# masnottuh/point-cloud-toolbox

Measured on AMD Instinct MI355X. Metric: points/sec curvature (1M-pt torus, k=50); HBM GB/s k-NN vs peak, higher is better.
Workload: dtype f64

## Files before the change

### point-cloud-toolbox_amd/csrc/pct_api.hip

```cpp
#include "pct_internal.h"
#include "pct_auto_route.h"
#include "pct_query_plan.h"
#include "pct_ball_plan.h"

#include <execinfo.h>
#include <math.h>
#include <mutex>
#include <signal.h>
#include <stdarg.h>
#include <stdlib.h>
#include <sys/prctl.h>
#include <unistd.h>

int pct_fail(pct_ctx* ctx, int code, const char* fmt, ...) {
    if (ctx) {
        va_list ap;
        va_start(ap, fmt);
        vsnprintf(ctx->err, sizeof(ctx->err), fmt, ap);
        va_end(ap);
    }
    return code;
}

extern char** environ;
// ... 182 lines not shown
    }
    for (auto& e : ctx->ev)
        if (hipEventCreate(&e) != hipSuccess) {
            delete ctx;
            return PCT_ERR_HIP;
        }
    for (int i = PCT_EV_CALL_BEGIN; i <= PCT_EV_FAST_END; ++i)
        if (hipEventCreate(&ctx->ev_prev[i]) != hipSuccess) {
            delete ctx;
            return PCT_ERR_HIP;
        }
    if (hipHostMalloc((void**)&ctx->pin, 4096, hipHostMallocMapped) != hipSuccess) {
        delete ctx;
        return PCT_ERR_OOM;
    }
    memset(ctx->pin, 0, 4096);
    if (hipDeviceGetAttribute(&ctx->clock_khz, hipDeviceAttributeWallClockRate, device) != hipSuccess || ctx->clock_khz < 0) ctx->clock_khz = 0;
    (void)hipGetLastError();
    *out = ctx;
    return PCT_OK;
}

void pct_destroy(pct_ctx* ctx) {
    if (!ctx) return;
    (void)hipSetDevice(ctx->device);
    if (ctx->stream) (void)hipStreamSynchronize(ctx->stream);
    pct_comm_release(ctx);
    pct_buf* all[] = {&ctx->xyz, &ctx->pts4, &ctx->pts4d, &ctx->cell_of, &ctx->cell_cnt, &ctx->cell_fill,
                      &ctx->scan_tmp, &ctx->occ, &ctx->redo, &ctx->row_of, &ctx->owned_pos, &ctx->cell_own, &ctx->cell_oth, &ctx->own_start, &ctx->sorted4, &ctx->sorted4d, &ctx->red, &ctx->nbr_pos,
                      &ctx->nbr_dist, &ctx->nbr_cnt, &ctx->counters, &ctx->coefs, &ctx->K, &ctx->H, &ctx->H2,
                      &ctx->stage_a, &ctx->stage_b, &ctx->stage_c, &ctx->stage_d, &ctx->row_done, &ctx->redo_m, &ctx->flag_buf, &ctx->dens_buf, &ctx->pub_pos, &ctx->pub_dist, &ctx->pub_cnt, &ctx->qpts4, &ctx->qry, &ctx->ball_off, &ctx->ball_idx, &ctx->ball_alt, &ctx->ball_dist, &ctx->fit_flag, &ctx->lvl_src,
                      &ctx->tree_codes, &ctx->tree_vals, &ctx->tree_lvl, &ctx->tree_head, &ctx->tree_marks, &ctx->tree_seg, &ctx->tree_runs, &ctx->tree_range, &ctx->tree_bucket, &ctx->tree_tmp,
                      &ctx->pca, &ctx->pca_aux, &ctx->pca_nbr, &ctx->pca_orig,
                      &ctx->bin_rec, &ctx->bin_mat, &ctx->bin_plan, &ctx->bin_base,
                      &ctx->area, &ctx->area_closed, &ctx->area_nverts, &ctx->area_over, &ctx->stamp_tickets};
    for (pct_buf* b : all) pct_release(b);
    if (ctx->pin) (void)hipHostFree(ctx->pin);
    for (auto& e : ctx->ev)
        if (e) (void)hipEventDestroy(e);
    for (auto& e : ctx->ev_prev)
        if (e) (void)hipEventDestroy(e);
    if (ctx->stream) (void)hipStreamDestroy(ctx->stream);
    delete ctx;
}

const char* pct_last_error(const pct_ctx* ctx) { return ctx ? ctx->err : "null context"; }

static int begin_call(pct_ctx* ctx, bool wait_for_pending = true) {
    if (!ctx) return PCT_ERR_INVALID;
    ctx->err[0] = 0;
    PCT_HIP(ctx, hipSetDevice(ctx->device));
    if (wait_for_pending) PCT_TRY(drain(ctx));
    return PCT_OK;
}

static int new_cloud(pct_ctx* ctx, int64_t n) {
    if (n <= 0 || n > (int64_t)INT32_MAX - 1024) return pct_fail(ctx, PCT_ERR_INVALID, "cloud size %lld out of range", (long long)n);
    ctx->n = n;
    ctx->q_begin = 0;
    ctx->q_end = n;
    ctx->slab_parts = ctx->slab_part = 0;
    ctx->slab_split_valid = false;
    ctx->grid_valid = ctx->knn_valid = ctx->fit_valid = ctx->pts4_valid = ctx->qpts4_valid = false;
    ctx->pca_valid = false;
    ctx->ball_valid = false;
    ctx->area_valid = false;
    ctx->has_f64 = false;
// ... 1202 lines not shown
```

### point-cloud-toolbox_amd/csrc/pct_grid.hip

```cpp
#include "pct_internal.h"
#include "pct_grid_edge.h"

#include <math.h>
#include <stdlib.h>

namespace {

constexpr int kBlock = 256;

__device__ __forceinline__ float wave_min(float v) {
    for (int o = 32; o > 0; o >>= 1) v = fminf(v, __shfl_xor(v, o));
    return v;
}
__device__ __forceinline__ float wave_max(float v) {
    for (int o = 32; o > 0; o >>= 1) v = fmaxf(v, __shfl_xor(v, o));
    return v;
}

struct PackRed {
    int bb[6];
    int bad;
    int g_begin;
    double s[3], ss[3];
    unsigned long long cnt;
// ... 798 lines not shown
__global__ __launch_bounds__(kBinWide) void k_bin_scatter(const float* __restrict__ xyz, const float4* __restrict__ pts4, int64_t n,
                                                           int tile_rows, pct_grid g, int shift, int nb, int chunk,
                                                           const unsigned* __restrict__ mat, const int* __restrict__ plan,
                                                           float4* __restrict__ rec, int* __restrict__ cell_own, int* __restrict__ cell_oth) {
    __shared__ unsigned s_cur[kBinMaxBuckets];
    const int* bstart = plan + 16;
    for (int b = threadIdx.x; b < nb; b += kBinWide) s_cur[b] = (unsigned)bstart[b] + mat[(size_t)blockIdx.x * nb + b];
    __syncthreads();
    const int64_t r0 = (int64_t)blockIdx.x * tile_rows, r1 = min(n, r0 + tile_rows);
    for (int64_t base = r0 + threadIdx.x; base < r1; base += 4 * kBinWide) {
        float4 p[4];
#pragma unroll
        for (int j = 0; j < 4; ++j)
            if (base + j * kBinWide < r1) p[j] = bin_load<RAW>(xyz, pts4, base + j * kBinWide);
#pragma unroll
        for (int j = 0; j < 4; ++j) {
            if (base + j * kBinWide >= r1) continue;
            const unsigned pos = atomicAdd(&s_cur[bin_cell(p[j].x, p[j].y, p[j].z, g) >> shift], 1u);
            if (pos < (unsigned)n) rec[pos] = p[j];
        }
    }
    if (plan[2] > 0) {
        for (int b = blockIdx.x; b < nb; b += gridDim.x) {
            if (bstart[b + 1] - bstart[b] <= chunk) continue;
            const int64_t c0 = (int64_t)b << shift, c1 = min(g.ncell, c0 + ((int64_t)1 << shift));
            for (int64_t c = c0 + threadIdx.x; c < c1; c += kBinWide) {
                cell_own[c] = 0;
                if (cell_oth) cell_oth[c] = 0;
            }
        }
    }
}

__global__ __launch_bounds__(kBinBlock) void k_bin_cells(const float4* __restrict__ rec, const int* __restrict__ plan,
                                                         const int4* __restrict__ items, pct_grid g, int shift, int q_begin, int q_end,
                                                         int* __restrict__ cell_own, int* __restrict__ cell_oth, int* __restrict__ base,
                                                         const PackRed* __restrict__ parts, int n_parts, PackRed* __restrict__ red,
                                                         PackRed* __restrict__ red_host) {
    extern __shared__ int s_c[];
    if (blockIdx.x == gridDim.x - 1) {
        if (parts) pack_fold<kBinBlock>(parts, n_parts, red, red_host, 0);
        return;
    }
    if ((int)blockIdx.x >= plan[0]) return;
    const int4 it = items[blockIdx.x];
    const int r0 = it.y, r1 = it.z, slot = it.w;
    const int cpb = 1 << shift, nc = cell_oth ? 2 * cpb : cpb;
    const int64_t c0 = (int64_t)it.x << shift;
    const int ncl = (int)min((int64_t)cpb, g.ncell - c0);
    for (int k = threadIdx.x; k < nc; k += kBinBlock) s_c[k] = 0;
    __syncthreads();
    for (int base = r0 + threadIdx.x; base < r1; base += 4 * kBinBlock) {
        float4 p[4];
#pragma unroll
        for (int j = 0; j < 4; ++j)
            if (base + j * kBinBlock < r1) p[j] = rec[base + j * kBinBlock];
#pragma unroll
        for (int j = 0; j < 4; ++j) {
            if (base + j * kBinBlock >= r1) continue;
            const int l = bin_cell(p[j].x, p[j].y, p[j].z, g) - (int)c0;
            const int idx = __float_as_int(p[j].w);
            const bool owned = !cell_oth || (idx >= q_begin && idx < q_end);
            if ((unsigned)l < (unsigned)cpb) atomicAdd(&s_c[(owned ? 0 : cpb) + l], 1);
        }
    }
    __syncthreads();
    for (int k = threadIdx.x; k < nc; k += kBinBlock) {
        const int l = k & (cpb - 1);
        if (l >= ncl) continue;
        int* arr = k < cpb ? cell_own : cell_oth;
        const int v = s_c[k];
        if (slot < 0) arr[c0 + l] = v;
        else base[(size_t)slot * nc + k] = v ? atomicAdd(&arr[c0 + l], v) : 0;
    }
}

__global__ __launch_bounds__(kBinBlock) void k_bin_place(const float4* __restrict__ rec, const int* __restrict__ plan,
                                                         const int4* __restrict__ items, pct_grid g, int shift, int q_begin, int q_end,
                                                         int64_t n, int64_t n_owned, const int* __restrict__ cell_start,
                                                         const int* __restrict__ cell_own, const int* __restrict__ cell_oth,
                                                         const int* __restrict__ own_start, const int* __restrict__ base,
                                                         float4* __restrict__ sorted4, int* __restrict__ row_of, int* __restrict__ owned_pos,
                                                         const double4* __restrict__ pts4d, double4* __restrict__ sorted4d) {
    extern __shared__ int s_cur[];
    if ((int)blockIdx.x >= plan[0]) return;
    const int4 it = items[blockIdx.x];
    const int r0 = it.y, r1 = it.z, slot = it.w;
    if (r0 >= r1) return;
    const int cpb = 1 << shift, nc = cell_oth ? 2 * cpb : cpb;
    const int64_t c0 = (int64_t)it.x << shift;
    const int ncl = (int)min((int64_t)cpb, g.ncell - c0);
    int* s_row = s_cur + nc;
    for (int k = threadIdx.x; k < nc; k += kBinBlock) {
        const int l = k & (cpb - 1);
        if (l >= ncl) continue;
        int s = cell_start[c0 + l];
        if (k >= cpb) s += cell_own[c0 + l];
        else if (cell_oth) s_row[l] = own_start[c0 + l] - s;
        if (slot >= 0) s += base[(size_t)slot * nc + k];
        s_cur[k] = s;
    }
    __syncthreads();
    for (int base = r0 + threadIdx.x; base < r1; base += 4 * kBinBlock) {
        float4 p[4];
#pragma unroll
        for (int j = 0; j < 4; ++j)
            if (base + j * kBinBlock < r1) p[j] = rec[base + j * kBinBlock];
#pragma unroll
        for (int j = 0; j < 4; ++j) {
            if (base + j * kBinBlock >= r1) continue;
            const int l = bin_cell(p[j].x, p[j].y, p[j].z, g) - (int)c0;
            const int idx = __float_as_int(p[j].w);
            const bool owned = !cell_oth || (idx >= q_begin && idx < q_end);
            if ((unsigned)l >= (unsigned)ncl) continue;
            const int pos = atomicAdd(&s_cur[(owned ? 0 : cpb) + l], 1);
            if ((unsigned)pos >= (unsigned)n) continue;
            sorted4[pos] = p[j];
            if (pts4d) sorted4d[pos] = pts4d[idx];
            if (owned) {
                const int row = cell_oth ? pos + s_row[l] : pos;
                if ((unsigned)row < (unsigned)n_owned && (unsigned)(idx - q_begin) < (unsigned)n_owned) {
                    owned_pos[row] = pos;
                    if (row_of) row_of[idx - q_begin] = row;
                }
            }
        }
    }
}

__global__ __launch_bounds__(256) void k_bin_row_of(const float4* __restrict__ sorted4, const int* __restrict__ owned_pos, int64_t n_owned,
                                                    int q_begin, int* __restrict__ row_of) {
    const int64_t row = (int64_t)blockIdx.x * 256 + threadIdx.x;
    if (row >= n_owned) return;
    const int idx = __float_as_int(sorted4[owned_pos[row]].w);
    if ((unsigned)(idx - q_begin) < (unsigned)n_owned) row_of[idx - q_begin] = (int)row;
}

__global__ __launch_bounds__(256) void k_gather_int(const int* __restrict__ map, int* __restrict__ io, int64_t n) {
    const int64_t i = (int64_t)blockIdx.x * 256 + threadIdx.x;
    if (i < n) io[i] = map[io[i]];
}

int grid_1d(int64_t n, int per_block, int cap) {
    int64_t b = (n + per_block - 1) / per_block;
    if (b < 1) b = 1;
    if (cap > 0 && b > cap) b = cap;
    return (int)b;
}

}

static PackRed* red_parts(pct_ctx* ctx) { return (PackRed*)((char*)ctx->red.p + 128); }
static_assert(sizeof(PackRed) <= sizeof(pct_pinned::pack_red) && alignof(PackRed) <= 128, "pct_pinned::pack_red holds a PackRed");
// ... 332 lines not shown
    PCT_TRY(pct_reserve(ctx, &ctx->cell_fill, (size_t)n * sizeof(int)));
    PCT_TRY(pct_reserve(ctx, &ctx->sorted4, (size_t)n * sizeof(float4)));
    PCT_TRY(pct_reserve(ctx, &ctx->row_of, (size_t)((ctx->own_flag ? n : n_owned) + 1) * sizeof(int)));
    PCT_TRY(pct_reserve(ctx, &ctx->owned_pos, (size_t)n_owned * sizeof(int)));
    if (ctx->has_f64) PCT_TRY(pct_reserve(ctx, &ctx->sorted4d, (size_t)n * sizeof(double4)));
    return PCT_OK;
}

static EdgeSearch edge_search(const pct_ctx* ctx, const GridPoints& s, double target, double eps) {
    EdgeSearch es = {};
    es.target = target; es.n = s.n; es.eps = eps;
    es.ex = (double)s.bbox[3] - s.bbox[0]; es.ey = (double)s.bbox[4] - s.bbox[1]; es.ez = (double)s.bbox[5] - s.bbox[2];
    es.hint_edge = ctx->hint_edge; es.hint_guess = ctx->hint_guess; es.hint_target = ctx->hint_target;
    es.level_edge = ctx->level_edge;
    es.max_iter = es.level_edge > 0 ? 1 : ctx->level_mode ? 2 : 8;
    return es;
}

enum class GridBuild {
    Bin,
    AtomicRaw,
    AtomicBase,
    AtomicPacked,
};
static GridBuild choose_build(bool bin_allowed, const BinShape& bs, const GridPoints& s) {
    return bin_allowed && bs.ok ? GridBuild::Bin : s.raw ? GridBuild::AtomicRaw : s.from_base ? GridBuild::AtomicBase : GridBuild::AtomicPacked;
}

struct BinScratch {
    int* plan;
    unsigned* tot;
    int4* items;
    size_t lds;
};
static int bin_scratch(pct_ctx* ctx, const BinShape& bs, int64_t n, BinScratch* b) {
    PCT_TRY(pct_reserve(ctx, &ctx->bin_rec, (size_t)n * sizeof(float4)));
    PCT_TRY(pct_reserve(ctx, &ctx->bin_mat, (size_t)bs.ntiles * bs.nb * sizeof(unsigned)));
    const size_t plan_words = 16 + (size_t)(bs.nb + 1) + (size_t)bs.nb;
    const size_t items_at = (plan_words * sizeof(int) + 15) / 16 * 16;
    PCT_TRY(pct_reserve(ctx, &ctx->bin_plan, items_at + (size_t)bs.max_items * sizeof(int4)));
    PCT_TRY(pct_reserve(ctx, &ctx->bin_base, (size_t)bs.max_shared * (bs.cls << bs.shift) * sizeof(int)));
    b->plan = (int*)ctx->bin_plan.p;
    b->tot = (unsigned*)(b->plan + 16 + bs.nb + 1);
    b->items = (int4*)((char*)ctx->bin_plan.p + items_at);
    b->lds = (size_t)(bs.cls << bs.shift) * sizeof(int);
    return PCT_OK;
}

struct GridPass {
    GridBuild build;
    pct_grid g;
    BinShape bs;
    BinScratch bin;
    const float4* src;
    int64_t n_owned;
    bool sharded, sub_box;
};

template <bool RAW>
static void launch_bin_count(pct_ctx* ctx, int64_t n, const GridPass& p, PackRed* parts, unsigned long long* begin_stamp) {
    PCT_LAUNCH_T(k_bin_count<RAW>, dim3(p.bs.ntiles), dim3(kBinWide), 0, ctx->stream, ctx->xyz_view, p.src, n, p.bs.tile_rows, p.g, p.bs.shift,
                 p.bs.nb, (unsigned*)ctx->bin_mat.p, parts, begin_stamp);
}
template <bool RAW>
static void launch_bin_scatter(pct_ctx* ctx, int64_t n, const GridPass& p, int* cell_oth) {
    PCT_LAUNCH_T(k_bin_scatter<RAW>, dim3(p.bs.ntiles), dim3(kBinWide), 0, ctx->stream, ctx->xyz_view, p.src, n, p.bs.tile_rows, p.g, p.bs.shift,
                 p.bs.nb, p.bs.chunk, (const unsigned*)ctx->bin_mat.p, (const int*)p.bin.plan, (float4*)ctx->bin_rec.p, (int*)ctx->cell_own.p, cell_oth);
}

static int launch_count(pct_ctx* ctx, const GridPoints& s, GridPass& p, CallBegin* begin) {
    const pct_grid& g = p.g;
    const int64_t n = s.n;
    const float* own_flag = (const float*)ctx->own_flag;
    const bool bin = p.build == GridBuild::Bin;
    PCT_TRY(pct_reserve(ctx, &ctx->cell_own, (size_t)g.ncell * sizeof(int)));
    if (begin && !bin) PCT_HIP(ctx, begin->fall_back(ctx->stream));
    if (!bin) PCT_HIP(ctx, hipMemsetAsync(ctx->cell_own.p, 0, (size_t)g.ncell * sizeof(int), ctx->stream));
    if (p.sharded) {
        PCT_TRY(pct_reserve(ctx, &ctx->cell_oth, (size_t)g.ncell * sizeof(int)));
        if (!bin) PCT_HIP(ctx, hipMemsetAsync(ctx->cell_oth.p, 0, (size_t)g.ncell * sizeof(int), ctx->stream));
    }
    if (bin) PCT_TRY(bin_scratch(ctx, p.bs, n, &p.bin));
    int* cell_oth = p.sharded ? (int*)ctx->cell_oth.p : nullptr;
    PackRed* parts = s.deferred_box ? red_parts(ctx) : nullptr;
    const int nhb = grid_1d(n, kBlock, 0);
    if (bin) {
        const BinShape& bs = p.bs;
        unsigned long long* begin_stamp = begin ? begin->take() : nullptr;
        s.raw ? launch_bin_count<true>(ctx, n, p, parts, begin_stamp) : launch_bin_count<false>(ctx, n, p, parts, begin_stamp);
        PCT_LAUNCH(k_bin_colscan, dim3((bs.nb + kBinScanCols - 1) / kBinScanCols), dim3(kBinScanCols * kBinScanGroups), 0, ctx->stream,
                   (unsigned*)ctx->bin_mat.p, bs.ntiles, bs.nb, p.bin.tot);
        PCT_LAUNCH(k_bin_plan, dim3(1), dim3(1024), 0, ctx->stream, (const unsigned*)p.bin.tot, bs.nb, bs.chunk, p.bin.plan, p.bin.items);
        s.raw ? launch_bin_scatter<true>(ctx, n, p, cell_oth) : launch_bin_scatter<false>(ctx, n, p, cell_oth);
        PCT_LAUNCH(k_bin_cells, dim3(bs.max_items + 1), dim3(kBinBlock), p.bin.lds, ctx->stream, (const float4*)ctx->bin_rec.p, (const int*)p.bin.plan,
                   (const int4*)p.bin.items, g, bs.shift, (int)ctx->q_begin, (int)ctx->q_end, (int*)ctx->cell_own.p, cell_oth,
                   (int*)ctx->bin_base.p, (const PackRed*)parts, bs.ntiles, (PackRed*)ctx->red.p, pin_red(ctx));
    } else if (p.build == GridBuild::AtomicRaw) {
        PCT_LAUNCH(k_hist_raw, dim3(nhb), dim3(kBlock), 0, ctx->stream, ctx->xyz_view, n, g, s.g_begin, s.g_end, (int*)ctx->cell_of.p,
                   (int*)ctx->cell_fill.p, (int*)ctx->cell_own.p, cell_oth, parts);
        if (parts) PCT_TRY(red_fold(ctx, nhb, false));
    } else if (p.build == GridBuild::AtomicBase) {
        PCT_LAUNCH(k_hist_agg, dim3(nhb), dim3(kBlock), 0, ctx->stream, p.src, n, g, own_flag, ctx->own_lo, ctx->own_hi, p.sub_box ? 1 : 0,
                   (int*)ctx->cell_of.p, (int*)ctx->cell_fill.p, (int*)ctx->cell_own.p, (int*)ctx->cell_oth.p);
    } else {
        PCT_LAUNCH(k_hist, dim3(nhb), dim3(kBlock), 0, ctx->stream, p.src, n, g, s.g_begin, s.g_end, own_flag, ctx->own_lo, ctx->own_hi,
                   p.sub_box ? 1 : 0, (int*)ctx->cell_of.p, (int*)ctx->cell_fill.p, (int*)ctx->cell_own.p, cell_oth);
    }
    return PCT_OK;
}

static int launch_scan(pct_ctx* ctx, const GridPass& p, int items_q, int nblk) {
    const int* cell_oth = p.sharded ? (const int*)ctx->cell_oth.p : nullptr;
    PCT_TRY(pct_reserve(ctx, &ctx->scan_tmp, (size_t)(nblk + 1) * sizeof(int4) + (size_t)nblk * sizeof(unsigned long long)));
    unsigned long long* sq_part = (unsigned long long*)((int4*)ctx->scan_tmp.p + nblk + 1);
    PCT_TRY(pct_reserve(ctx, &ctx->cell_cnt, (size_t)(p.g.ncell + 1) * sizeof(int)));
    PCT_TRY(pct_reserve(ctx, &ctx->own_start, (size_t)(p.g.ncell + 1) * sizeof(int)));
    PCT_TRY(pct_reserve(ctx, &ctx->occ, ((size_t)(p.n_owned < p.g.ncell ? p.n_owned : p.g.ncell) + (size_t)p.n_owned / items_q + 16) * sizeof(int2)));
    PCT_LAUNCH(k_scan_sums, dim3(nblk), dim3(kBlock), 0, ctx->stream, (const int*)ctx->cell_own.p, cell_oth, p.g.ncell, items_q,
               (int4*)ctx->scan_tmp.p, sq_part);
    PCT_TRY(pct_reserve(ctx, &ctx->counters, sizeof(pct_dev_words)));
    PCT_LAUNCH(k_scan_tiles, dim3(1), dim3(1024), 0, ctx->stream, (int4*)ctx->scan_tmp.p, nblk,
               (const unsigned long long*)sq_part, pin_totals(ctx), (unsigned long long*)&pct_dev(ctx)->sweep);
    ctx->counters_clean = true;
    PCT_HIP(ctx, hipEventRecord(ctx->ev[PCT_EV_SCAN_TOTALS], ctx->stream));
    PCT_LAUNCH(k_scan_apply, dim3(nblk), dim3(kBlock), 0, ctx->stream, (const int*)ctx->cell_own.p, cell_oth, p.g.ncell, items_q,
               (const int4*)ctx->scan_tmp.p, (int*)ctx->cell_cnt.p, (int*)ctx->own_start.p, (int2*)ctx->occ.p);
    return PCT_OK;
}

static int launch_place(pct_ctx* ctx, const GridPoints& s, const GridPass& p) {
    const pct_grid& g = p.g;
    const int64_t n = s.n;
    const bool lazy_rows = p.build == GridBuild::Bin && !ctx->level_mode;
    ctx->row_of_valid = !lazy_rows;
    ctx->row_of_rows = p.n_owned;
    ctx->row_of_begin = (int)ctx->q_begin;
    const int* cell_oth = p.sharded ? (const int*)ctx->cell_oth.p : nullptr;
    const double4* pts4d = ctx->has_f64 ? (const double4*)ctx->pts4d.p : nullptr;
    double4* sorted4d = ctx->has_f64 ? (double4*)ctx->sorted4d.p : nullptr;
    if (p.build == GridBuild::Bin)
        PCT_LAUNCH(k_bin_place, dim3(p.bs.max_items), dim3(kBinBlock), p.bin.lds + (p.sharded ? p.bin.lds / 2 : 0), ctx->stream,
                   (const float4*)ctx->bin_rec.p, (const int*)p.bin.plan, (const int4*)p.bin.items, g, p.bs.shift, (int)ctx->q_begin,
                   (int)ctx->q_end, n, p.n_owned, (const int*)ctx->cell_cnt.p, (const int*)ctx->cell_own.p, cell_oth,
                   (const int*)ctx->own_start.p, (const int*)ctx->bin_base.p, (float4*)ctx->sorted4.p,
                   lazy_rows ? nullptr : (int*)ctx->row_of.p, (int*)ctx->owned_pos.p, pts4d, sorted4d);
    else if (p.build == GridBuild::AtomicRaw)
        PCT_LAUNCH(k_scatter_raw, dim3(grid_1d(n, kBlock, 0)), dim3(kBlock), 0, ctx->stream, ctx->xyz_view, (const int*)ctx->cell_of.p,
                   (const int*)ctx->cell_cnt.p, (const int*)ctx->cell_own.p, (const int*)ctx->own_start.p, (const int*)ctx->cell_fill.p, n,
                   s.g_begin, (float4*)ctx->sorted4.p, (int*)ctx->row_of.p, (int*)ctx->owned_pos.p, pts4d, sorted4d);
    else
        PCT_LAUNCH(k_scatter, dim3(grid_1d(n, kBlock, 0)), dim3(kBlock), 0, ctx->stream, p.src, (const int*)ctx->cell_of.p,
                   (const int*)ctx->cell_cnt.p, (const int*)ctx->cell_own.p, (const int*)ctx->own_start.p, (const int*)ctx->cell_fill.p, n,
                   s.g_begin, (float4*)ctx->sorted4.p, (int*)ctx->row_of.p, (int*)ctx->owned_pos.p, pts4d, sorted4d);
    PCT_HIP(ctx, hipGetLastError());
    return PCT_OK;
}

static int debug_bin_plan(pct_ctx* ctx, const GridPass& p) {
    int pw[3] = {0, 0, 0};
    PCT_HIP(ctx, hipMemcpyAsync(pw, p.bin.plan, sizeof(pw), hipMemcpyDeviceToHost, ctx->stream));
    PCT_HIP(ctx, hipStreamSynchronize(ctx->stream));
    fprintf(stderr, "[grid] bin build: %d buckets of %d cells, %d tiles of %d rows, %d work items of up to %d records, %d of them in %d shared buckets\n",
            p.bs.nb, 1 << p.bs.shift, p.bs.ntiles, p.bs.tile_rows, pw[0], p.bs.chunk, pw[1], pw[2]);
    return PCT_OK;
}

static int commit_grid(pct_ctx* ctx, const GridPoints& s, pct_grid g, const EdgeSearch& es, int iters, double m_last, int4 tot,
                       int64_t n_owned, bool sub_box) {
    const bool own_flag = ctx->own_flag != nullptr, level_pass = es.level_edge > 0;
    const int64_t n = s.n;
    for (int ax = 0; ax < 3; ++ax) {
        const double o = ax == 0 ? g.ox : ax == 1 ? g.oy : g.oz;
        g.lim_lo[ax] = ctx->culled ? ((double)s.kept_box.lo[ax] - o) * g.inv_cell : -INFINITY;
        g.lim_hi[ax] = ctx->culled ? ((double)s.kept_box.hi[ax] - o) * g.inv_cell : INFINITY;
    }
    if (pct_getenv("PCT_GRID_DEBUG"))
        fprintf(stderr, "[grid] box [%g %g %g]-[%g %g %g] edge %g dims %d x %d x %d = %lld cells, %d passes, occupancy %.1f, items %d\n", s.bbox[0],
                s.bbox[1], s.bbox[2], s.bbox[3], s.bbox[4], s.bbox[5], g.cell, g.nx, g.ny, g.nz, (long long)g.ncell, iters, m_last, tot.y);
// ... 16 lines not shown
        ctx->hint_edge = es.hint_after(g.cell, m_last);
        ctx->hint_guess = es.first_guess;
        ctx->hint_target = es.target;
    }
    if ((tot.x != n && !sub_box) || tot.x > n || tot.z != n_owned)
        return pct_fail(ctx, PCT_ERR_INVALID, "cell scan totals %d/%d != %lld/%lld", tot.x, tot.z, (long long)n, (long long)n_owned);
    if (!level_pass && m_last > 64.0 * es.target && m_last * 27.0 * (double)n_owned > 1e12)
        return pct_fail(ctx, PCT_ERR_INVALID,
                        "the cell list cannot resolve this cloud: a point shares its cell with %.0f others on average at the "
                        "smallest usable cell edge %.3g (%lld cells); thin it out or split it into compact pieces",
                        m_last, g.cell, (long long)g.ncell);
    ctx->n_items = tot.y;
    ctx->nonempty_cells = tot.w;
    ctx->n_occ = tot.y;
    ctx->tm.occupied_cells = tot.y;
    ctx->grid_valid = true;
    ctx->grid_whole = !own_flag && !ctx->level_mode && !sub_box && !ctx->culled && n == ctx->n && ctx->q_begin == 0 && ctx->q_end == ctx->n &&
                      ctx->slab_parts == 0;
    return PCT_OK;
}

int pct_build_grid(pct_ctx* ctx, int32_t k, double eps, bool may_give_up, GridVerdict* out, CallBegin* begin) {
    *out = GridVerdict::Built;
    ctx->grid_valid = false;
    const double factor = ctx->occupancy_factor > 0 ? ctx->occupancy_factor : pct_default_factor(k);
    const double target = factor * (k + 1);
    int64_t cell_cap = (int64_t)1 << 27;
    if (ctx->level_mode) cell_cap = (int64_t)1 << 24;
    else if (32 * ctx->n > cell_cap) cell_cap = 32 * ctx->n < ((int64_t)1 << 30) ? 32 * ctx->n : (int64_t)1 << 30;
    const bool own_flag = ctx->own_flag != nullptr;
    const bool slab = ctx->slab_parts >= 1 && !own_flag;
    const bool sub_box = ctx->level_edge > 0 && ctx->level_box_valid;
    const bool bin_allowed = !own_flag && !sub_box && !slab && !pct_getenv("PCT_GRID_ATOMIC");
    int items_q = 16;
    if (const char* e = pct_getenv("PCT_ITEMS_Q")) { const int v = atoi(e); if (v >= 1 && v <= 64) items_q = v; }

    for (int attempt = 0; attempt < 3; ++attempt) {
        ctx->tm.grid_iters = 0;
        if (slab) PCT_TRY(slab_split(ctx));
        const int64_t n_owned = own_flag ? ctx->own_count : ctx->q_end - ctx->q_begin;
        const bool sharded = own_flag || ctx->q_begin > 0 || ctx->q_end < ctx->n || slab;
        GridPoints s;
        bool restart = false;
        PCT_TRY(select_source(ctx, k, target, slab, n_owned, sharded, &s, &restart, begin));
        if (restart) continue;
        const int64_t n = s.n;
        ctx->items_q = items_q;
        PCT_TRY(reserve_lists(ctx, n, n_owned));
        EdgeSearch es = edge_search(ctx, s, target, eps);
        double a = es.first();
        GridPass p = {};
        p.src = s.from_base ? (const float4*)ctx->lvl_src.p : (const float4*)ctx->pts4.p;
        p.n_owned = n_owned; p.sharded = sharded; p.sub_box = sub_box;
        int iters = 0;
        int4 tot = make_int4(0, 0, 0, 0);
        double m_last = 0;
        for (int it = 0; it < es.max_iter; ++it) {
            a = es.clamp_eps(a);
            size_grid(ctx, sub_box, s.bbox, a, &p.g);
            if (!own_flag && !(es.level_edge > 0) && p.g.ncell > 16 * n && p.g.ncell > ((int64_t)1 << 20)) {
                if (it == 0 && es.hinted) {
                    a = es.fallback_first();
                    size_grid(ctx, sub_box, s.bbox, a, &p.g);
                } else if (may_give_up) {
                    *out = GridVerdict::GaveUp;
                    ctx->grid_valid = false;
                    return PCT_OK;
                }
            }
            bool hit_cap = false;
            while (p.g.ncell > cell_cap) {
                a *= cbrt((double)p.g.ncell / (double)cell_cap) * 1.01;
                size_grid(ctx, sub_box, s.bbox, a, &p.g);
                hit_cap = true;
            }
            const pct_grid& g = p.g;
            p.bs = bin_allowed ? bin_shape(n, g.ncell, sharded) : BinShape{};
            p.build = choose_build(bin_allowed, p.bs, s);
            const bool bin = p.build == GridBuild::Bin;
            PCT_TRY(launch_count(ctx, s, p, begin));
            const int nblk = (int)((g.ncell + kScanTile - 1) / kScanTile);
            if (pct_getenv("PCT_GRID_DEBUG"))
                fprintf(stderr, "[grid] pass %d: n %lld owned %lld edge %g dims %d x %d x %d = %lld cells (%d scan tiles), box [%g %g %g]-[%g %g %g]\n", it,
                        (long long)n, (long long)n_owned, a, g.nx, g.ny, g.nz, (long long)g.ncell, nblk, s.bbox[0], s.bbox[1], s.bbox[2], s.bbox[3], s.bbox[4], s.bbox[5]);
            PCT_TRY(launch_scan(ctx, p, items_q, nblk));
            PCT_TRY(launch_place(ctx, s, p));
            PCT_HIP(ctx, hipEventSynchronize(ctx->ev[PCT_EV_SCAN_TOTALS]));
            if (s.deferred_box) {
                const BoxCheck box = check_deferred_box(ctx, &s);
                if (box == BoxCheck::NonFinite) return pct_fail(ctx, PCT_ERR_NONFINITE, "Non-finite values in input points");
                if (box == BoxCheck::Restart) {
                    ctx->spec_valid = false;
                    restart = true;
                    break;
                }
            }
            if (bin && pct_getenv("PCT_GRID_DEBUG")) PCT_TRY(debug_bin_plan(ctx, p));
            tot = pin_totals(ctx)->tot;
            m_last = (double)pin_totals(ctx)->sumsq / (double)(n_owned > 0 ? n_owned : 1);
            ++iters;
            if (es.accept(m_last, a, g.ncell, cell_cap, hit_cap, it)) break;
            a = es.next(m_last, a);
        }
        if (restart) continue;
        return commit_grid(ctx, s, p.g, es, iters, m_last, tot, n_owned, sub_box);
    }
    return pct_fail(ctx, PCT_ERR_INVALID, "cell-list build: restarted more than twice");
}

int pct_ensure_row_of(pct_ctx* ctx) {
    if (ctx->row_of_valid) return PCT_OK;
    const int64_t rows = ctx->row_of_rows;
// ... 15 lines not shown
```

### point-cloud-toolbox_amd/csrc/pct_grid_edge.h

```cpp
#pragma once

#include <math.h>
#include <stdint.h>

struct EdgeSearch {
    double target;
    int64_t n;
    double ex, ey, ez;
    double eps;
    double hint_edge, hint_guess, hint_target;
    double level_edge;
    int max_iter;
    double emax = 1.0;
    double first_guess = 0;
    bool hinted = false;
    double a_prev = 0, m_prev = 0, d_last = 2.0;

    static constexpr double kWinLo = 0.88, kWinHi = 1.12;

    double cap() const { return emax * 1.0001 + 1e-30; }

    double first() {
        emax = fmax(ex, fmax(ey, ez));
        if (!(emax > 0)) emax = 1.0;
// ... 50 lines not shown
constexpr int kBinMaxCounters = 8192;
constexpr int kBinMinChunk = 4096;

struct BinShape {
    bool ok;
    int shift;
    int nb;
    int cls;
    int tile_rows, ntiles;
    int chunk;
    int max_items;
    int max_shared;
};

inline BinShape bin_shape(int64_t n, int64_t ncell, bool sharded) {
    BinShape s = {};
    s.cls = sharded ? 2 : 1;
    int max_shift = 8;
    while ((s.cls << (max_shift + 1)) <= kBinMaxCounters) ++max_shift;
    s.shift = 8;
    while (((ncell + ((int64_t)1 << s.shift) - 1) >> s.shift) > 1024 && s.shift < max_shift) ++s.shift;
    const int64_t nb = (ncell + ((int64_t)1 << s.shift) - 1) >> s.shift;
    s.ok = n >= 1 && n < ((int64_t)1 << 31) - kBinTileRows && ncell >= 1 && nb <= kBinMaxBuckets;
    if (!s.ok) return s;
    s.nb = (int)nb;
    const int64_t f = (n + (int64_t)kBinTileRows * kBinMaxTiles - 1) / ((int64_t)kBinTileRows * kBinMaxTiles);
    s.tile_rows = (int)(kBinTileRows * (f < 1 ? 1 : f));
    s.ntiles = (int)((n + s.tile_rows - 1) / s.tile_rows);
    s.chunk = (s.cls << s.shift) > kBinMinChunk ? (s.cls << s.shift) : kBinMinChunk;
    s.max_items = s.nb + (int)(n / s.chunk);
    s.max_shared = 2 * (int)(n / s.chunk) + 1;
    return s;
}
```

### point-cloud-toolbox_amd/csrc/pct_internal.h

```cpp
#pragma once

#include <hip/hip_runtime.h>
#include <stdint.h>
#include <stdio.h>
#include <string.h>
#include <stdlib.h>

#include "../../include/pct_hip.h"
#include "pct_stamp.h"

#define PCT_WAVE 64
#define PCT_K_MAX 511

extern const char* pct_last_launch;
#define PCT_STR2(x) #x
#define PCT_STR(x) PCT_STR2(x)
#define PCT_LAUNCH(kernelName, ...)                                                          \
    do {                                                                                     \
        __atomic_store_n(&pct_last_launch, __FILE__ ":" PCT_STR(__LINE__) "  " #kernelName, __ATOMIC_RELAXED); \
        hipLaunchKernelGGL((kernelName), __VA_ARGS__);                                       \
    } while (0)
const char* pct_launch_name(const char* where, const char* instantiation);
#define PCT_LAUNCH_T(kernelName, ...)                                                        \
    do {                                                                                     \
// ... 136 lines not shown
    pct_buf tree_seg, tree_runs;
    pct_buf tree_range;
    pct_buf tree_bucket;
    pct_buf tree_tmp;
    pct_buf row_done;
    pct_buf redo_m;
    pct_buf flag_buf;
    pct_buf dens_buf;
    pct_buf pub_pos, pub_dist, pub_cnt;
    float tree_bbox[6] = {0, 0, 0, 0, 0, 0};
    int64_t auto_tree_n = 0;
    int32_t auto_tree_calls = 0;
    float auto_tree_bbox[6] = {0, 0, 0, 0, 0, 0};
    bool has_f64 = false;
    double occupancy_factor = 0.0;
    bool collect_stats = false;

    pct_buf xyz;
    const float* xyz_view = nullptr;
    pct_buf pts4;
    pct_buf pts4d;
    pct_grid grid = {};
    pct_buf cell_of;
    pct_buf cell_cnt;
    pct_buf cell_own;
    pct_buf cell_oth;
    pct_buf own_start;
    pct_buf cell_fill;
    pct_buf scan_tmp;
    pct_buf bin_rec;
    pct_buf bin_mat;
    pct_buf bin_plan;
    pct_buf bin_base;
    pct_buf occ;
    pct_buf redo;
    int64_t n_items = 0;
    int64_t nonempty_cells = 0;
    int32_t items_q = 12;
    pct_buf sorted4;
    pct_buf sorted4d;
    pct_buf row_of;
    bool row_of_valid = true;
    int64_t row_of_rows = 0;
    int32_t row_of_begin = 0;
    pct_buf owned_pos;
    pct_buf red;
    pct_pinned* pin = nullptr;
    int64_t n_occ = 0;
    bool grid_valid = false;
    bool grid_whole = false;
    bool pts4_valid = false;

    pct_buf nbr_pos;
    pct_buf nbr_dist;
    pct_buf nbr_cnt;
    int32_t k = 0;
    int32_t nbr_pitch = 0;
    double eps = 0.0;
    bool counters_clean = false;
    int fit_parity = 0;
    void* fit_flag_seen = nullptr;
    size_t fit_flag_cap_seen = 0;
    bool knn_valid = false;
    bool knn_hier = false;
    bool knn_sorted_space = false;
    bool dist_valid = true;
// ... 197 lines not shown
```

Baseline: 1.498 billion.

## Fuse grid prefix scan into bin kernels via per-bucket sums and tickets

k_bin_cells now computes per-bucket totals (counts, items, owned, occupied, squared sum). For shared buckets, a last-arriving-block ticket decides which block does this. k_bin_place then does the in-bucket exclusive scan itself, writes cell_start/own_start and the occ list, so the separate global k_scan_sums pass over all cells is skipped and only a small tile scan over buckets remains. LDS counters are padded to avoid bank conflicts, and the first record loads are hoisted ahead of the scan. This trades a full-grid scan pass for extra work and atomics inside the binning kernels, and adds ticket-based cross-block synchronisation.

```diff
diff --git a/point-cloud-toolbox_amd/csrc/pct_api.hip b/point-cloud-toolbox_amd/csrc/pct_api.hip
--- a/point-cloud-toolbox_amd/csrc/pct_api.hip
+++ b/point-cloud-toolbox_amd/csrc/pct_api.hip
@@ -238,7 +238,7 @@
                       &ctx->stage_a, &ctx->stage_b, &ctx->stage_c, &ctx->stage_d, &ctx->row_done, &ctx->redo_m, &ctx->flag_buf, &ctx->dens_buf, &ctx->pub_pos, &ctx->pub_dist, &ctx->pub_cnt, &ctx->qpts4, &ctx->qry, &ctx->ball_off, &ctx->ball_idx, &ctx->ball_alt, &ctx->ball_dist, &ctx->fit_flag, &ctx->lvl_src,
                       &ctx->tree_codes, &ctx->tree_vals, &ctx->tree_lvl, &ctx->tree_head, &ctx->tree_marks, &ctx->tree_seg, &ctx->tree_runs, &ctx->tree_range, &ctx->tree_bucket, &ctx->tree_tmp,
                       &ctx->pca, &ctx->pca_aux, &ctx->pca_nbr, &ctx->pca_orig,
-                      &ctx->bin_rec, &ctx->bin_mat, &ctx->bin_plan, &ctx->bin_base,
+                      &ctx->bin_rec, &ctx->bin_mat, &ctx->bin_plan, &ctx->bin_base, &ctx->bin_sums,
                       &ctx->area, &ctx->area_closed, &ctx->area_nverts, &ctx->area_over, &ctx->stamp_tickets};
     for (pct_buf* b : all) pct_release(b);
     if (ctx->pin) (void)hipHostFree(ctx->pin);
diff --git a/point-cloud-toolbox_amd/csrc/pct_grid.hip b/point-cloud-toolbox_amd/csrc/pct_grid.hip
--- a/point-cloud-toolbox_amd/csrc/pct_grid.hip
+++ b/point-cloud-toolbox_amd/csrc/pct_grid.hip
@@ -854,11 +854,17 @@
     }
 }
 
+__device__ __forceinline__ int bin_items(int o, int items_q, unsigned magic) {
+    return magic && o < (1 << 24) ? (int)__umulhi((unsigned)(o + items_q - 1), magic) : (o + items_q - 1) / items_q;
+}
+__host__ __device__ __forceinline__ int bin_pad(int l) { return l + (l >> 5); }
+
 __global__ __launch_bounds__(kBinBlock) void k_bin_cells(const float4* __restrict__ rec, const int* __restrict__ plan,
                                                          const int4* __restrict__ items, pct_grid g, int shift, int q_begin, int q_end,
                                                          int* __restrict__ cell_own, int* __restrict__ cell_oth, int* __restrict__ base,
                                                          const PackRed* __restrict__ parts, int n_parts, PackRed* __restrict__ red,
-                                                         PackRed* __restrict__ red_host) {
+                                                         PackRed* __restrict__ red_host, int items_q, unsigned q_magic, int chunk, int4* __restrict__ bsum,
+                                                         unsigned long long* __restrict__ bsq, unsigned* __restrict__ ticket) {
     extern __shared__ int s_c[];
     if (blockIdx.x == gridDim.x - 1) {
         if (parts) pack_fold<kBinBlock>(parts, n_parts, red, red_host, 0);
@@ -895,39 +901,147 @@
         if (slot < 0) arr[c0 + l] = v;
         else base[(size_t)slot * nc + k] = v ? atomicAdd(&arr[c0 + l], v) : 0;
     }
+    if (!bsum) return;
+    __shared__ int s_last;
+    if (slot >= 0) {
+        asm volatile("s_waitcnt vmcnt(0)" ::: "memory");
+        __syncthreads();
+        if (threadIdx.x == 0) {
+            const int* bstart = plan + 16;
+            const unsigned ni = (unsigned)((bstart[it.x + 1] - bstart[it.x] + chunk - 1) / chunk);
+            unsigned* tk = ticket + (size_t)it.x * kBinTicketWords;
+            const unsigned t = __hip_atomic_fetch_add(tk, 1u, __ATOMIC_RELAXED, __HIP_MEMORY_SCOPE_AGENT);
+            s_last = t + 1u == ni;
+            if (t + 1u == ni) __hip_atomic_store(tk, 0u, __ATOMIC_RELAXED, __HIP_MEMORY_SCOPE_AGENT);
+        }
+        __syncthreads();
+        if (!s_last) return;
+    }
+    int4 v = make_int4(0, 0, 0, 0);
+    unsigned long long sq = 0;
+    for (int l = threadIdx.x; l < ncl; l += kBinBlock) {
+        int o, t;
+        if (slot < 0) {
+            o = s_c[l];
+            t = o + (cell_oth ? s_c[cpb + l] : 0);
+        } else {
+            o = __hip_atomic_load(&cell_own[c0 + l], __ATOMIC_RELAXED, __HIP_MEMORY_SCOPE_AGENT);
+            t = o + (cell_oth ? __hip_atomic_load(&cell_oth[c0 + l], __ATOMIC_RELAXED, __HIP_MEMORY_SCOPE_AGENT) : 0);
+        }
+        v = add3(v, make_int4(t, bin_items(o, items_q, q_magic), o, t > 0 ? 1 : 0));
+        sq += (unsigned long long)o * (unsigned)t;
+    }
+    __shared__ int4 s_v[kBinBlock / 64];
+    __shared__ unsigned long long s_q[kBinBlock / 64];
+    for (int o = 32; o > 0; o >>= 1) {
+        v.x += __shfl_xor(v.x, o); v.y += __shfl_xor(v.y, o); v.z += __shfl_xor(v.z, o); v.w += __shfl_xor(v.w, o);
+        sq += __shfl_xor(sq, o);
+    }
+    if ((threadIdx.x & 63) == 0) {
+        s_v[threadIdx.x >> 6] = v;
+        s_q[threadIdx.x >> 6] = sq;
+    }
+    __syncthreads();
+    if (threadIdx.x == 0) {
+        for (int i = 1; i < kBinBlock / 64; ++i) { v = add3(v, s_v[i]); sq += s_q[i]; }
+        bsum[it.x] = v;
+        bsq[it.x] = sq;
+    }
 }
 
 __global__ __launch_bounds__(kBinBlock) void k_bin_place(const float4* __restrict__ rec, const int* __restrict__ plan,
-                                                         const int4* __restrict__ items, pct_grid g, int shift, int q_begin, int q_end,
-                                                         int64_t n, int64_t n_owned, const int* __restrict__ cell_start,
+                                                         const int4* __restrict__ items, pct_grid g, int shift, int nb, int q_begin, int q_end,
+                                                         int64_t n, int64_t n_owned, int* __restrict__ cell_start,
                                                          const int* __restrict__ cell_own, const int* __restrict__ cell_oth,
-                                                         const int* __restrict__ own_start, const int* __restrict__ base,
+                                                         int* __restrict__ own_start, const int* __restrict__ base,
                                                          float4* __restrict__ sorted4, int* __restrict__ row_of, int* __restrict__ owned_pos,
-                                                         const double4* __restrict__ pts4d, double4* __restrict__ sorted4d) {
+                                                         const double4* __restrict__ pts4d, double4* __restrict__ sorted4d,
+                                                         int items_q, unsigned q_magic, const int4* __restrict__ bsum, int2* __restrict__ occ) {
     extern __shared__ int s_cur[];
     if ((int)blockIdx.x >= plan[0]) return;
     const int4 it = items[blockIdx.x];
     const int r0 = it.y, r1 = it.z, slot = it.w;
-    if (r0 >= r1) return;
-    const int cpb = 1 << shift, nc = cell_oth ? 2 * cpb : cpb;
+    const bool first = bsum && (slot < 0 || r0 == plan[16 + it.x]);
+    if (r0 >= r1 && !first) return;
+    const int cpb = 1 << shift, nc = cell_oth ? 2 * cpb : cpb, P = bin_pad(cpb);
     const int64_t c0 = (int64_t)it.x << shift;
     const int ncl = (int)min((int64_t)cpb, g.ncell - c0);
-    int* s_row = s_cur + nc;
-    for (int k = threadIdx.x; k < nc; k += kBinBlock) {
-        const int l = k & (cpb - 1);
-        if (l >= ncl) continue;
-        int s = cell_start[c0 + l];
-        if (k >= cpb) s += cell_own[c0 + l];
-        else if (cell_oth) s_row[l] = own_start[c0 + l] - s;
-        if (slot >= 0) s += base[(size_t)slot * nc + k];
-        s_cur[k] = s;
+    int* s_oth = s_cur + P;
+    int* s_row = s_cur + (cell_oth ? 2 * P : P);
+    float4 p[4];
+#pragma unroll
+    for (int j = 0; j < 4; ++j)
+        if (r0 + (int)threadIdx.x + j * kBinBlock < r1) p[j] = rec[r0 + threadIdx.x + j * kBinBlock];
+    if (bsum) {
+        const int4 bb = bsum[it.x];
+        for (int l = threadIdx.x; l < cpb; l += kBinBlock) {
+            s_cur[bin_pad(l)] = l < ncl ? cell_own[c0 + l] : 0;
+            if (cell_oth) s_oth[bin_pad(l)] = l < ncl ? cell_oth[c0 + l] : 0;
+        }
+        __syncthreads();
+        const int per = cpb / kBinBlock, l0 = bin_pad(threadIdx.x * per);
+        int vx = 0, vy = 0, vz = 0;
+        for (int j = 0; j < per; ++j) {
+            const int o = s_cur[l0 + j];
+            vx += o + (cell_oth ? s_oth[l0 + j] : 0);
+            vy += bin_items(o, items_q, q_magic);
+            vz += o;
+        }
+        int ix = vx, iy = vy, iz = vz;
+        const int lane = threadIdx.x & 63, wv = threadIdx.x >> 6;
+        for (int o = 1; o < 64; o <<= 1) {
+            const int tx = __shfl_up(ix, o), ty = __shfl_up(iy, o), tz = __shfl_up(iz, o);
+            if (lane >= o) { ix += tx; iy += ty; iz += tz; }
+        }
+        __shared__ int s_w[kBinBlock / 64][3];
+        if (lane == 63) { s_w[wv][0] = ix; s_w[wv][1] = iy; s_w[wv][2] = iz; }
+        __syncthreads();
+        for (int i = 0; i < wv; ++i) { ix += s_w[i][0]; iy += s_w[i][1]; iz += s_w[i][2]; }
+        int s = bb.x + ix - vx, r = bb.y + iy - vy, w = bb.z + iz - vz;
+        for (int j = 0; j < per; ++j) {
+            const int o = s_cur[l0 + j], ot = cell_oth ? s_oth[l0 + j] : 0;
+            if (first) {
+                const int ni = bin_items(o, items_q, q_magic);
+                for (int ch = 0; ch < ni; ++ch) occ[r++] = make_int2((int)(c0 + threadIdx.x * per + j), ch);
+            }
+            s_cur[l0 + j] = s;
+            if (cell_oth) {
+                s_oth[l0 + j] = s + o;
+                s_row[l0 + j] = w - s;
+            }
+            s += o + ot;
+            w += o;
+        }
+        if (first && it.x == nb - 1 && threadIdx.x == kBinBlock - 1) { cell_start[g.ncell] = s; own_start[g.ncell] = w; }
+        __syncthreads();
+        for (int l = threadIdx.x; l < ncl; l += kBinBlock) {
+            const int cs = s_cur[bin_pad(l)];
+            if (first) {
+                cell_start[c0 + l] = cs;
+                own_start[c0 + l] = cell_oth ? cs + s_row[bin_pad(l)] : cs;
+            }
+            if (slot >= 0) {
+                s_cur[bin_pad(l)] = cs + base[(size_t)slot * nc + l];
+                if (cell_oth) s_oth[bin_pad(l)] += base[(size_t)slot * nc + cpb + l];
+            }
+        }
+    } else {
+        for (int l = threadIdx.x; l < ncl; l += kBinBlock) {
+            const int cs = cell_start[c0 + l], off = slot >= 0 ? base[(size_t)slot * nc + l] : 0;
+            s_cur[bin_pad(l)] = cs + off;
+            if (cell_oth) {
+                s_oth[bin_pad(l)] = cs + cell_own[c0 + l] + (slot >= 0 ? base[(size_t)slot * nc + cpb + l] : 0);
+                s_row[bin_pad(l)] = own_start[c0 + l] - cs;
+            }
+        }
     }
     __syncthreads();
     for (int base = r0 + threadIdx.x; base < r1; base += 4 * kBinBlock) {
-        float4 p[4];
-#pragma unroll
-        for (int j = 0; j < 4; ++j)
-            if (base + j * kBinBlock < r1) p[j] = rec[base + j * kBinBlock];
+        if (base != r0 + (int)threadIdx.x) {
+#pragma unroll
+            for (int j = 0; j < 4; ++j)
+                if (base + j * kBinBlock < r1) p[j] = rec[base + j * kBinBlock];
+        }
 #pragma unroll
         for (int j = 0; j < 4; ++j) {
             if (base + j * kBinBlock >= r1) continue;
@@ -935,12 +1049,12 @@
             const int idx = __float_as_int(p[j].w);
             const bool owned = !cell_oth || (idx >= q_begin && idx < q_end);
             if ((unsigned)l >= (unsigned)ncl) continue;
-            const int pos = atomicAdd(&s_cur[(owned ? 0 : cpb) + l], 1);
+            const int pos = atomicAdd(&s_cur[(owned ? 0 : P) + bin_pad(l)], 1);
             if ((unsigned)pos >= (unsigned)n) continue;
             sorted4[pos] = p[j];
             if (pts4d) sorted4d[pos] = pts4d[idx];
             if (owned) {
-                const int row = cell_oth ? pos + s_row[l] : pos;
+                const int row = cell_oth ? pos + s_row[bin_pad(l)] : pos;
                 if ((unsigned)row < (unsigned)n_owned && (unsigned)(idx - q_begin) < (unsigned)n_owned) {
                     owned_pos[row] = pos;
                     if (row_of) row_of[idx - q_begin] = row;
@@ -1339,6 +1453,9 @@
     unsigned* tot;
     int4* items;
     size_t lds;
+    unsigned* ticket;
+    int4* bsum;
+    unsigned long long* bsq;
 };
 static int bin_scratch(pct_ctx* ctx, const BinShape& bs, int64_t n, BinScratch* b) {
     PCT_TRY(pct_reserve(ctx, &ctx->bin_rec, (size_t)n * sizeof(float4)));
@@ -1351,6 +1468,13 @@
     b->tot = (unsigned*)(b->plan + 16 + bs.nb + 1);
     b->items = (int4*)((char*)ctx->bin_plan.p + items_at);
     b->lds = (size_t)(bs.cls << bs.shift) * sizeof(int);
+    const BinSums bl = bin_sums_layout(bs);
+    const size_t cap_before = ctx->bin_sums.cap;
+    PCT_TRY(pct_reserve(ctx, &ctx->bin_sums, bl.bytes));
+    if (ctx->bin_sums.cap != cap_before) PCT_HIP(ctx, hipMemsetAsync(ctx->bin_sums.p, 0, bl.slots_at, ctx->stream));
+    b->ticket = (unsigned*)((char*)ctx->bin_sums.p + bl.tickets_at);
+    b->bsum = (int4*)((char*)ctx->bin_sums.p + bl.slots_at);
+    b->bsq = (unsigned long long*)((char*)ctx->bin_sums.p + bl.sq_at);
     return PCT_OK;
 }
 
@@ -1362,6 +1486,9 @@
     const float4* src;
     int64_t n_owned;
     bool sharded, sub_box;
+    bool bucket_scan;
+    int items_q;
+    unsigned q_magic;
 };
 
 template <bool RAW>
@@ -1401,7 +1528,8 @@
         s.raw ? launch_bin_scatter<true>(ctx, n, p, cell_oth) : launch_bin_scatter<false>(ctx, n, p, cell_oth);
         PCT_LAUNCH(k_bin_cells, dim3(bs.max_items + 1), dim3(kBinBlock), p.bin.lds, ctx->stream, (const float4*)ctx->bin_rec.p, (const int*)p.bin.plan,
                    (const int4*)p.bin.items, g, bs.shift, (int)ctx->q_begin, (int)ctx->q_end, (int*)ctx->cell_own.p, cell_oth,
-                   (int*)ctx->bin_base.p, (const PackRed*)parts, bs.ntiles, (PackRed*)ctx->red.p, pin_red(ctx));
+                   (int*)ctx->bin_base.p, (const PackRed*)parts, bs.ntiles, (PackRed*)ctx->red.p, pin_red(ctx), p.items_q, p.q_magic, bs.chunk,
+                   p.bucket_scan ? p.bin.bsum : nullptr, p.bin.bsq, p.bin.ticket);
     } else if (p.build == GridBuild::AtomicRaw) {
         PCT_LAUNCH(k_hist_raw, dim3(nhb), dim3(kBlock), 0, ctx->stream, ctx->xyz_view, n, g, s.g_begin, s.g_end, (int*)ctx->cell_of.p,
                    (int*)ctx->cell_fill.p, (int*)ctx->cell_own.p, cell_oth, parts);
@@ -1418,14 +1546,21 @@
 
 static int launch_scan(pct_ctx* ctx, const GridPass& p, int items_q, int nblk) {
     const int* cell_oth = p.sharded ? (const int*)ctx->cell_oth.p : nullptr;
-    PCT_TRY(pct_reserve(ctx, &ctx->scan_tmp, (size_t)(nblk + 1) * sizeof(int4) + (size_t)nblk * sizeof(unsigned long long)));
-    unsigned long long* sq_part = (unsigned long long*)((int4*)ctx->scan_tmp.p + nblk + 1);
     PCT_TRY(pct_reserve(ctx, &ctx->cell_cnt, (size_t)(p.g.ncell + 1) * sizeof(int)));
     PCT_TRY(pct_reserve(ctx, &ctx->own_start, (size_t)(p.g.ncell + 1) * sizeof(int)));
     PCT_TRY(pct_reserve(ctx, &ctx->occ, ((size_t)(p.n_owned < p.g.ncell ? p.n_owned : p.g.ncell) + (size_t)p.n_owned / items_q + 16) * sizeof(int2)));
+    PCT_TRY(pct_reserve(ctx, &ctx->counters, sizeof(pct_dev_words)));
+    if (p.bucket_scan) {
+        PCT_LAUNCH(k_scan_tiles, dim3(1), dim3(1024), 0, ctx->stream, p.bin.bsum, p.bs.nb, (const unsigned long long*)p.bin.bsq, pin_totals(ctx),
+                   (unsigned long long*)&pct_dev(ctx)->sweep);
+        ctx->counters_clean = true;
+        PCT_HIP(ctx, hipEventRecord(ctx->ev[PCT_EV_SCAN_TOTALS], ctx->stream));
+        return PCT_OK;
+    }
+    PCT_TRY(pct_reserve(ctx, &ctx->scan_tmp, (size_t)(nblk + 1) * sizeof(int4) + (size_t)nblk * sizeof(unsigned long long)));
+    unsigned long long* sq_part = (unsigned long long*)((int4*)ctx->scan_tmp.p + nblk + 1);
     PCT_LAUNCH(k_scan_sums, dim3(nblk), dim3(kBlock), 0, ctx->stream, (const int*)ctx->cell_own.p, cell_oth, p.g.ncell, items_q,
                (int4*)ctx->scan_tmp.p, sq_part);
-    PCT_TRY(pct_reserve(ctx, &ctx->counters, sizeof(pct_dev_words)));
     PCT_LAUNCH(k_scan_tiles, dim3(1), dim3(1024), 0, ctx->stream, (int4*)ctx->scan_tmp.p, nblk,
                (const unsigned long long*)sq_part, pin_totals(ctx), (unsigned long long*)&pct_dev(ctx)->sweep);
     ctx->counters_clean = true;
@@ -1446,11 +1581,12 @@
     const double4* pts4d = ctx->has_f64 ? (const double4*)ctx->pts4d.p : nullptr;
     double4* sorted4d = ctx->has_f64 ? (double4*)ctx->sorted4d.p : nullptr;
     if (p.build == GridBuild::Bin)
-        PCT_LAUNCH(k_bin_place, dim3(p.bs.max_items), dim3(kBinBlock), p.bin.lds + (p.sharded ? p.bin.lds / 2 : 0), ctx->stream,
-                   (const float4*)ctx->bin_rec.p, (const int*)p.bin.plan, (const int4*)p.bin.items, g, p.bs.shift, (int)ctx->q_begin,
-                   (int)ctx->q_end, n, p.n_owned, (const int*)ctx->cell_cnt.p, (const int*)ctx->cell_own.p, cell_oth,
-                   (const int*)ctx->own_start.p, (const int*)ctx->bin_base.p, (float4*)ctx->sorted4.p,
-                   lazy_rows ? nullptr : (int*)ctx->row_of.p, (int*)ctx->owned_pos.p, pts4d, sorted4d);
+        PCT_LAUNCH(k_bin_place, dim3(p.bs.max_items), dim3(kBinBlock), (size_t)(p.sharded ? 3 : 1) * bin_pad(1 << p.bs.shift) * sizeof(int), ctx->stream,
+                   (const float4*)ctx->bin_rec.p, (const int*)p.bin.plan, (const int4*)p.bin.items, g, p.bs.shift, p.bs.nb, (int)ctx->q_begin,
+                   (int)ctx->q_end, n, p.n_owned, (int*)ctx->cell_cnt.p, (const int*)ctx->cell_own.p, cell_oth,
+                   (int*)ctx->own_start.p, (const int*)ctx->bin_base.p, (float4*)ctx->sorted4.p,
+                   lazy_rows ? nullptr : (int*)ctx->row_of.p, (int*)ctx->owned_pos.p, pts4d, sorted4d, p.items_q, p.q_magic,
+                   p.bucket_scan ? (const int4*)p.bin.bsum : nullptr, (int2*)ctx->occ.p);
     else if (p.build == GridBuild::AtomicRaw)
         PCT_LAUNCH(k_scatter_raw, dim3(grid_1d(n, kBlock, 0)), dim3(kBlock), 0, ctx->stream, ctx->xyz_view, (const int*)ctx->cell_of.p,
                    (const int*)ctx->cell_cnt.p, (const int*)ctx->cell_own.p, (const int*)ctx->own_start.p, (const int*)ctx->cell_fill.p, n,
@@ -1533,6 +1669,7 @@
     const bool slab = ctx->slab_parts >= 1 && !own_flag;
     const bool sub_box = ctx->level_edge > 0 && ctx->level_box_valid;
     const bool bin_allowed = !own_flag && !sub_box && !slab && !pct_getenv("PCT_GRID_ATOMIC");
+    const bool bucket_scan = !pct_getenv("PCT_GRID_GLOBAL_SCAN");
     int items_q = 16;
     if (const char* e = pct_getenv("PCT_ITEMS_Q")) { const int v = atoi(e); if (v >= 1 && v <= 64) items_q = v; }
 
@@ -1552,7 +1689,8 @@
         double a = es.first();
         GridPass p = {};
         p.src = s.from_base ? (const float4*)ctx->lvl_src.p : (const float4*)ctx->pts4.p;
-        p.n_owned = n_owned; p.sharded = sharded; p.sub_box = sub_box;
+        p.n_owned = n_owned; p.sharded = sharded; p.sub_box = sub_box; p.items_q = items_q;
+        p.q_magic = items_q >= 2 ? (unsigned)(0x100000000ull / (unsigned)items_q) + 1u : 0u;
         int iters = 0;
         int4 tot = make_int4(0, 0, 0, 0);
         double m_last = 0;
@@ -1579,6 +1717,7 @@
             p.bs = bin_allowed ? bin_shape(n, g.ncell, sharded) : BinShape{};
             p.build = choose_build(bin_allowed, p.bs, s);
             const bool bin = p.build == GridBuild::Bin;
+            p.bucket_scan = bin && bucket_scan;
             PCT_TRY(launch_count(ctx, s, p, begin));
             const int nblk = (int)((g.ncell + kScanTile - 1) / kScanTile);
             if (pct_getenv("PCT_GRID_DEBUG"))
diff --git a/point-cloud-toolbox_amd/csrc/pct_grid_edge.h b/point-cloud-toolbox_amd/csrc/pct_grid_edge.h
--- a/point-cloud-toolbox_amd/csrc/pct_grid_edge.h
+++ b/point-cloud-toolbox_amd/csrc/pct_grid_edge.h
@@ -106,3 +106,16 @@
     s.max_shared = 2 * (int)(n / s.chunk) + 1;
     return s;
 }
+
+constexpr int kBinTicketWords = 32;
+struct BinSums {
+    size_t tickets_at, slots_at, sq_at, bytes;
+};
+inline BinSums bin_sums_layout(const BinShape& s) {
+    BinSums l = {};
+    l.tickets_at = 0;
+    l.slots_at = (size_t)kBinMaxBuckets * kBinTicketWords * sizeof(unsigned);
+    l.sq_at = l.slots_at + ((size_t)s.nb + 1) * 16;
+    l.bytes = l.sq_at + (size_t)s.nb * sizeof(unsigned long long);
+    return l;
+}
diff --git a/point-cloud-toolbox_amd/csrc/pct_internal.h b/point-cloud-toolbox_amd/csrc/pct_internal.h
--- a/point-cloud-toolbox_amd/csrc/pct_internal.h
+++ b/point-cloud-toolbox_amd/csrc/pct_internal.h
@@ -192,6 +192,7 @@
     pct_buf bin_mat;
     pct_buf bin_plan;
     pct_buf bin_base;
+    pct_buf bin_sums;
     pct_buf occ;
     pct_buf redo;
     int64_t n_items = 0;
```

Result: slower. 1.431 billion (-4.5%).
